# HKU-MedAI/WSI-HGNN

Hardware: AMD Instinct MI355X
Metric: edges/s fwd+bwd HEATNet4, 10k-node/6-rel synth graph, 1->8 MI355X (higher is better)
Workload: dtype f32 (fp16x3 emulation: 2-way fp16 split scaled per row (Y = XW^T, dX) or per column (dW), 3 products - bf16x6 for small launches; fp32-class error)

## Files before the change

### include/wsi_hgnn.h

```cpp
#ifndef WSI_HGNN_H
#define WSI_HGNN_H

#include <stdint.h>

#ifdef __cplusplus
extern "C" {
#endif

#define WSI_OK        0
#define WSI_EINVAL  (-22)
#define WSI_ENOSYS  (-38)
#define WSI_EFAULT  (-14)
#define WSI_ENOMEM  (-12)

#define WSI_ABI_VERSION 26

int         wsi_abi_version(void);
const char* wsi_last_error(void);

typedef struct wsi_context wsi_context_t;
int  wsi_context_create(wsi_context_t** out);
void wsi_context_destroy(wsi_context_t* ctx);

#define WSI_ATTN_XCD_CONTIGUOUS 1
#define WSI_ATTN_HUB_DEGREE(d) (((d) & 0xffff) << 8)
int wsi_heat_attn_fwd(const float* q, int64_t ldq, const float* k, int64_t ldk, const float* v, int64_t ldv,
                      int32_t num_nodes, int32_t D, int32_t H,
                      const int32_t* node_seg, const int32_t* rowptr, const int32_t* src, const float* sim,
                      const int32_t* order, int32_t num_heavy, int32_t flags,
                      const float* e_weight, const float* e_bias,
                      float* t, int64_t ldt, float* score, float* lse,
                      uint32_t* t_absmax,
                      wsi_context_t* ctx, void* stream);

int wsi_heat_attn_scores_fwd(const float* q, int64_t ldq, const float* k, int64_t ldk, int32_t num_nodes, int32_t D, int32_t H,
                             const int32_t* node_seg, const int32_t* rowptr, const int32_t* src, const float* sim,
                             const int32_t* order, int32_t num_heavy, int32_t flags, const float* e_weight, const float* e_bias,
                             float* score, float* lse, wsi_context_t* ctx, void* stream);

int wsi_heat_pool_coeff(const float* score, const float* lse, const int32_t* edge_seg,
                        const int32_t* colptr, const int32_t* csc_eid, const int32_t* csc_dst, const float* inv_rd,
                        const int32_t* row_seg, int32_t segs_per_type, int32_t n_types, int32_t H, int32_t num_src,
                        float* ctab, void* stream);

int wsi_heat_pool_gtab(const float* h, int64_t ldh, int32_t D, int32_t H, const float* y, const float* beta,
                       const int32_t* chunk_row, const int32_t* chunk_seg, int32_t num_chunks,
                       int32_t segs_per_type, int32_t n_types, float* gtab, void* stream);
// ... 176 lines not shown

int wsi_cross_entropy(const float* logits, const int64_t* labels, int32_t B, int32_t C, float* loss, float* dlogits, int32_t* bad_label, void* stream);

int wsi_segment_dot_diff(const float* g, int64_t ldg, const float* a, int64_t lda, const float* b, int64_t ldb,
                         int32_t D, const int32_t* chunk_row, int32_t num_chunks,
                         const int32_t* seg_chunk, int32_t num_segs,
                         float* partial, float* out, void* stream);

int wsi_gate_grad(const float* g, int64_t ldg, const float* a, int64_t lda, const float* b, int64_t ldb,
                  int32_t D, const int32_t* chunk_row, int32_t num_chunks, const int32_t* seg_chunk, int32_t num_segs,
                  const int32_t* seg_gate, const float* skip, int32_t n_gates, float* partial, float* g_skip, void* stream);

int wsi_pool_factors(const float* x, int64_t ldx, int32_t D, const float* w, int64_t ldw, int32_t T, int32_t H, int32_t Bg,
                     const int32_t* chunk_row, int32_t num_chunks, const int32_t* seg_chunk,
                     float* partial, float* hp, float* csum, float* x_mean, void* stream);
int wsi_pool_tmean(const float* tpart, int32_t T, int32_t S, int32_t D, int32_t H, const float* csum, const float* const* bv,
                   const float* scale, float* t_mean, void* stream);
int wsi_pool_bwd_prep(const float* g_pool, int32_t S, int32_t D, int32_t op, const float* counts, const float* z_mean, const float* h_mean,
                      const int32_t* seg_gate, const float* skip, int32_t n_gates, const int32_t* type_gate, int32_t T,
                      float* g_row, float* g_sum, float* g_skip, float* omg, void* stream);
int wsi_pool_bwd_bias(const float* gt_seg, int32_t T, int32_t S, int32_t D, int32_t H, const float* const* bv, const float* csum,
                      float* beta, float* gbv, void* stream);

int wsi_plan_assemble(const int64_t* desc, int32_t nsegs, int32_t total_blocks, void* stream);
int wsi_slot_fill(const int64_t* desc, int32_t nsegs, int32_t total_blocks, void* stream);

int wsi_layernorm_fwd(const float* x, int64_t ldx, int32_t n, int32_t D, float eps,
                      const float* gamma, const float* beta, const int32_t* row_param,
                      float* y, int64_t ldy, float* stats, void* stream);
int wsi_layernorm_bwd(const float* gy, int64_t ldgy, const float* x, int64_t ldx, int32_t n, int32_t D,
                      const float* gamma, const int32_t* row_param, const float* stats,
                      float* gx, int64_t ldgx, float* xhat_gy, int64_t ldp, void* stream);
int wsi_gelu_fwd(const float* x, float* y, int64_t n, void* stream);
int wsi_gelu_bwd(const float* x, const float* gy, float* gx, int64_t n, void* stream);
int wsi_spmm_sum(const float* x, int64_t ldx, int32_t n_out, int32_t D,
                 const int32_t* ptr, const int32_t* idx, const float* edge_w, const float* iscale, const float* oscale,
                 const float* bias, int32_t relu, const float* relu_ref, int64_t ldref,
                 float* out, int64_t ldo, void* stream);
int wsi_sddmm_dot(const float* g, int64_t ldg, const float* x, int64_t ldx, int32_t n, int32_t D,
                  const int32_t* rowptr, const int32_t* src, const float* iscale, const float* oscale,
                  const float* relu_ref, int64_t ldref, float* g_w, void* stream);

int wsi_row_sqnorm(const float* x, int64_t ldx, int32_t n, int32_t F, float* out, void* stream);
int wsi_knn_select(const float* dots, int64_t ldd, const float* sqnorm, int32_t row0, int32_t rows, int32_t N,
                   int32_t kc, int32_t* cand, void* stream);
int wsi_pair_stats(const float* x, int64_t ldx, int32_t n, int32_t F, const int32_t* cand, int32_t kc, int32_t keep,
// ... 83 lines not shown
```

### wsi-hgnn_amd/csrc/heat_attn.hip

```cpp
#include "common.h"
#include <math.h>
#include <stdlib.h>
#include <mutex>
#include <type_traits>
#include <new>

namespace wsi {

struct AttnGraph {
    const int32_t* node_seg;
    const int32_t* rowptr;
    const int32_t* src;
    const float* sim;
    const int32_t* order;
    int32_t num_nodes;
    int32_t heavy_n;
    int32_t pass;
    int32_t heavy_deg;
    int32_t xcd;
    uint32_t* absmax;
    const float* score_in;
    const int32_t* gt_row;
};

// ... 342 lines not shown
    const float* __restrict__ score, const float* __restrict__ lse, const int32_t* __restrict__ edge_seg,
    const int32_t* __restrict__ colptr, const int32_t* __restrict__ csc_eid, const int32_t* __restrict__ csc_dst,
    const float* __restrict__ inv_rd, const int32_t* __restrict__ row_seg, int32_t segs_per_type, int32_t n_types, int32_t H,
    int32_t num_src, float* __restrict__ ctab) {
    const int64_t idx = (int64_t)blockIdx.x * 256 + threadIdx.x;
    if (idx >= (int64_t)num_src * H) return;
    const int u = (int)(idx / H), h = (int)(idx - (int64_t)u * H);
    float cb[kPoolTypes];
#pragma unroll
    for (int b = 0; b < kPoolTypes; ++b) cb[b] = 0.f;
    const int j0 = colptr[u], j1 = colptr[u + 1];
    for (int j = j0; j < j1; ++j) {
        const int e = csc_eid[j], w = csc_dst[j];
        const float a = expf(score[(int64_t)e * H + h] - lse[(int64_t)edge_seg[e] * H + h]) * inv_rd[w];
        const int bin = row_seg[w] / segs_per_type;
#pragma unroll
        for (int b = 0; b < kPoolTypes; ++b) cb[b] += (bin == b) ? a : 0.f;
    }
#pragma unroll
    for (int b = 0; b < kPoolTypes; ++b)
        if (b < n_types) ctab[((int64_t)u * n_types + b) * H + h] = cb[b];
}

template <int V, int LPH, int U, bool COOP = false>
__global__ __launch_bounds__(kBlock) void heat_attn_bwd_p2_kernel(
    AttnTables tb, AttnGraph g, const float* __restrict__ e_weight, const float* __restrict__ e_bias,
    float inv_sqrt_dk, const float* __restrict__ a, const float* __restrict__ ga,
    float* __restrict__ gsc, float* __restrict__ gea, float* __restrict__ gq, int64_t ldgq) {
    constexpr int H = 64 / LPH;
    __shared__ float sm_acc[COOP ? kWavesPerBlock * 64 * V : 1];
    int lane;
    const int w = wave_uniform_node<COOP>(g, lane);
    if (w < 0) return;
    const int part = COOP ? (int)(threadIdx.x >> 6) : 0;
    constexpr int ESTEP = COOP ? kWavesPerBlock * U : U;
    const int head = lane / LPH;
    const bool leader = (lane % LPH) == 0;
    const int col = lane * V;

    float gqa[V];
#pragma unroll
    for (int i = 0; i < V; ++i) gqa[i] = 0.f;

    const int s0 = g.node_seg[w], s1 = g.node_seg[w + 1];
    if (s1 > s0 && g.rowptr[s0] != g.rowptr[s1]) {
        float q[V];
        load_vec<V>(q, tb.q + (int64_t)w * tb.ldq + col);
        const float we = *e_weight, be = *e_bias;
        for (int s = s0; s < s1; ++s) {
            const int e0 = g.rowptr[s], e1 = g.rowptr[s + 1];
            if (e0 == e1) continue;
            float delta = 0.f;
            for (int e = e0; e < e1; ++e) {
                const int64_t o = (int64_t)e * H + head;
                delta = fmaf(a[o], ga[o], delta);
            }
            for (int e = e0 + part * U; e < e1; e += ESTEP) {
                float kk[U][V];
                float c[U], aa[U], gg[U];
#pragma unroll
                for (int j = 0; j < U; ++j) {
                    if (e + j < e1) {
                        const int u = g.src[e + j];
                        c[j] = (we * g.sim[e + j] + be) * inv_sqrt_dk;
                        const int64_t o = (int64_t)(e + j) * H + head;
                        aa[j] = a[o];
                        gg[j] = ga[o];
                        load_vec<V>(kk[j], tb.k + (int64_t)u * tb.ldk + col);
                    }
                }
#pragma unroll
                for (int j = 0; j < U; ++j) {
                    if (e + j < e1) {
                        float d = 0.f;
#pragma unroll
                        for (int i = 0; i < V; ++i) d = fmaf(q[i], kk[j][i], d);
                        d = group_sum<LPH>(d);
                        const float gs = aa[j] * (gg[j] - delta);
                        const float gc = gs * c[j];
#pragma unroll
                        for (int i = 0; i < V; ++i) gqa[i] = fmaf(gc, kk[j][i], gqa[i]);
                        if (leader) {
                            const int64_t o = (int64_t)(e + j) * H + head;
                            gsc[o] = gc;
                            gea[o] = gs * d * inv_sqrt_dk;
                        }
                    }
                }
            }
        }
    }
    if constexpr (COOP) {
#pragma unroll
        for (int i = 0; i < V; ++i) sm_acc[(part * V + i) * 64 + lane] = gqa[i];
        __syncthreads();
        if (part != 0) return;
#pragma unroll
        for (int i = 0; i < V; ++i) {
            float x = 0.f;
#pragma unroll
// ... 25 lines not shown
    int u = order ? order[wave] : wave;
    u = __builtin_amdgcn_readfirstlane(u);
    const int head = lane / LPH;
    const int col = lane * V;

    float gka[V], gva[V];
#pragma unroll
    for (int i = 0; i < V; ++i) { gka[i] = 0.f; gva[i] = 0.f; }
    float cb[POOL ? kPoolTypes : 1];
#pragma unroll
    for (int b = 0; b < (POOL ? kPoolTypes : 1); ++b) cb[b] = 0.f;

    const int j0 = colptr[u], j1 = colptr[u + 1];
    for (int j = j0; j < j1; j += U) {
        float qq[U][V], gt[U][V];
        float aa[U], gg[U];
        int bin[U];
#pragma unroll
        for (int x = 0; x < U; ++x) {
            if (j + x < j1) {
                const int eid = csc_eid[j + x];
                const int w = csc_dst[j + x];
                const int64_t o = (int64_t)eid * H + head;
                if constexpr (!KONLY) aa[x] = a[o] * inv_rd[w];
                gg[x] = gsc[o];
                load_vec<V>(qq[x], qtab + (int64_t)w * ldq + col);
                if constexpr (POOL) bin[x] = pool.ctab_ready ? -1 : pool.row_seg[w] / pool.segs_per_type;
                else if constexpr (!KONLY) load_vec<V>(gt[x], g_t + (int64_t)(gt_row ? gt_row[w] : w) * ldgt + col);
            }
        }
#pragma unroll
        for (int x = 0; x < U; ++x) {
            if (j + x < j1) {
#pragma unroll
                for (int i = 0; i < V; ++i) {
                    gka[i] = fmaf(gg[x], qq[x][i], gka[i]);
                    if constexpr (!POOL && !KONLY) gva[i] = fmaf(aa[x], gt[x][i], gva[i]);
                }
                if constexpr (POOL) {
#pragma unroll
                    for (int b = 0; b < kPoolTypes; ++b) cb[b] += (bin[x] == b) ? aa[x] : 0.f;
                }
            }
        }
    }
    store_vec<V>(gk + (int64_t)u * ldgk + col, gka);
    if constexpr (POOL) {
        const int su = pool.row_seg[u];
        const int tu = su / pool.segs_per_type, gu = su - tu * pool.segs_per_type;
        float racc[V];
        load_vec<V>(racc, pool.g_row + (int64_t)su * (V * 64) + col);
        const float om = pool.omg[tu];
#pragma unroll
        for (int i = 0; i < V; ++i) racc[i] *= om;
        const float* ybase = pool.y + (int64_t)tu * pool.num_segs * H * (V * 64);
#pragma unroll
        for (int b = 0; b < kPoolTypes; ++b) {
            if (b < pool.n_types) {
                if (pool.ctab_ready) cb[b] = pool.ctab[((int64_t)u * pool.n_types + b) * H + head];
                const float* yrow = ybase + (int64_t)(b * pool.segs_per_type + gu) * H * (V * 64) + col;
#pragma unroll
                for (int h = 0; h < H; ++h) {
                    const float c = __shfl(cb[b], h * LPH, 64);
                    float yv[V];
// ... 489 lines not shown
        AttnGraph gh = g, gl = g;
        gh.pass = 2; gh.num_nodes = g.heavy_n;
        gl.pass = 1;
        SideStream* side;
        hipStream_t hs = hub_fork(st, ctx, side);
        hipLaunchKernelGGL((heat_attn_fwd_kernel<V, LPH, kHeavyUnroll, true, true>), dim3(g.heavy_n), dim3(kBlock), 0, hs,
                           tb, gh, ew, eb, isd, (float*)nullptr, (int64_t)0, score, lse);
        hipLaunchKernelGGL((heat_attn_fwd_kernel<V, LPH, U, false, true>), dim3(blocks), dim3(kBlock), 0, st,
                           tb, gl, ew, eb, isd, (float*)nullptr, (int64_t)0, score, lse);
        hub_join(st, side);
        return check_launch("heat_attn_scores_fwd");
    }
    hipLaunchKernelGGL((heat_attn_fwd_kernel<V, LPH, U, false, true>), dim3(blocks), dim3(kBlock), 0, st,
                       tb, g, ew, eb, isd, (float*)nullptr, (int64_t)0, score, lse);
    return check_launch("heat_attn_scores_fwd");
}

template <int V, int LPH>
int launch_bwd(const AttnTables& tb, const AttnGraph& gd, int32_t num_src, int32_t E,
               const int32_t* colptr, const int32_t* csc_eid, const int32_t* csc_dst, const float* inv_rd,
               const int32_t* order_src, const float* ew, const float* eb, float isd,
               const float* g_t, int64_t ldgt, float* score_a, const float* lse, float* ga, float* gsc, float* gea,
               float* red_ws, float* gq, int64_t ldgq, float* gk, int64_t ldgk, float* gv, int64_t ldgv,
               float* g_e, const AttnPool* pool, SideStream* ctx, hipStream_t st) {
    constexpr int U = Unroll<V, LPH>::value;
    constexpr int H = 64 / LPH;
    const int blocks = (gd.num_nodes + kWavesPerBlock - 1) / kWavesPerBlock;
    const int sblocks = (num_src + kWavesPerBlock - 1) / kWavesPerBlock;
    const bool ph = pool && pool->h;
    const bool pflat = pool && pool->gtab;
    const char* bwd_mode = knob("WSI_ATTN_BWD");
    const bool srcmajor = !pool && !(bwd_mode && bwd_mode[0] == 'd');
    if (srcmajor) {
        int32_t* edge_seg = reinterpret_cast<int32_t*>(gsc);
        if (E > 0)
            hipLaunchKernelGGL(heat_attn_edge_seg_kernel, dim3((unsigned)((E + 255) / 256)), dim3(256), 0, st, gd.node_seg, gd.rowptr, gd.num_nodes, E, edge_seg);
        if (sblocks > 0) {
            constexpr int UA = U;
            auto pass_a = [&](auto uu) {
                hipLaunchKernelGGL((heat_attn_bwd_srcA_kernel<V, LPH, decltype(uu)::value>), dim3(sblocks), dim3(kBlock), 0, st,
                                   tb.v, tb.ldv, g_t, ldgt, gd.gt_row, gd.node_seg, (const int32_t*)edge_seg, colptr, csc_eid, csc_dst, inv_rd,
                                   order_src, num_src, gd.xcd, gd.score_in, score_a, lse, ga, gv, ldgv, gd.absmax);
            };
#ifdef WSI_ABLATE
            const char* su = knob("WSI_ATTN_SRC_U");
            const int ua = su ? su[0] - '0' : UA;
            if (ua == 2) pass_a(std::integral_constant<int, 2>{});
            else if (ua == 4) pass_a(std::integral_constant<int, 4>{});
            else if (ua == 8) pass_a(std::integral_constant<int, 8>{});
            else pass_a(std::integral_constant<int, UA>{});
#else
            pass_a(std::integral_constant<int, UA>{});
#endif
        }
    }
    if (pflat && E > 0) {
        const int64_t EH = (int64_t)E * H;
        hipLaunchKernelGGL(heat_attn_bwd_p1_flat_kernel, dim3((unsigned)((EH + 255) / 256)), dim3(256), 0, st, gd.src, pool->edge_seg, pool->seg_dst,
                           pool->row_seg, pool->segs_per_type, pool->n_types, inv_rd, pool->gtab, lse, EH, (int32_t)H, gd.score_in, score_a, ga);
    }
    if (blocks > 0 && gd.heavy_n > 0) {
        AttnGraph gh = gd, gl = gd;
        gh.pass = 2; gh.num_nodes = gd.heavy_n;
        gl.pass = 1;
        const dim3 hb(gd.heavy_n);
        SideStream* side;
        hipStream_t hs = hub_fork(st, ctx, side);
        if (pflat || srcmajor) {}
        else if (ph) hipLaunchKernelGGL((heat_attn_bwd_p1_kernel<V, LPH, kHeavyUnroll, true, true>), hb, dim3(kBlock), 0, hs, tb, gh, g_t, ldgt, score_a, lse, ga, *pool);
        else hipLaunchKernelGGL((heat_attn_bwd_p1_kernel<V, LPH, kHeavyUnroll, true>), hb, dim3(kBlock), 0, hs, tb, gh, g_t, ldgt, score_a, lse, ga, AttnPool{});
        hipLaunchKernelGGL((heat_attn_bwd_p2_kernel<V, LPH, kHeavyUnroll, true>), hb, dim3(kBlock), 0, hs,
                           tb, gh, ew, eb, isd, (const float*)score_a, (const float*)ga, gsc, gea, gq, ldgq);
        if (pflat || srcmajor) {}
        else if (ph) hipLaunchKernelGGL((heat_attn_bwd_p1_kernel<V, LPH, U, false, true>), dim3(blocks), dim3(kBlock), 0, st, tb, gl, g_t, ldgt, score_a, lse, ga, *pool);
        else hipLaunchKernelGGL((heat_attn_bwd_p1_kernel<V, LPH, U>), dim3(blocks), dim3(kBlock), 0, st, tb, gl, g_t, ldgt, score_a, lse, ga, AttnPool{});
        hipLaunchKernelGGL((heat_attn_bwd_p2_kernel<V, LPH, U>), dim3(blocks), dim3(kBlock), 0, st,
                           tb, gl, ew, eb, isd, (const float*)score_a, (const float*)ga, gsc, gea, gq, ldgq);
        hub_join(st, side);
    } else if (blocks > 0) {
        if (pflat || srcmajor) {}
        else if (ph) hipLaunchKernelGGL((heat_attn_bwd_p1_kernel<V, LPH, U, false, true>), dim3(blocks), dim3(kBlock), 0, st,
                                        tb, gd, g_t, ldgt, score_a, lse, ga, *pool);
        else hipLaunchKernelGGL((heat_attn_bwd_p1_kernel<V, LPH, U>), dim3(blocks), dim3(kBlock), 0, st,
                                tb, gd, g_t, ldgt, score_a, lse, ga, AttnPool{});
        hipLaunchKernelGGL((heat_attn_bwd_p2_kernel<V, LPH, U>), dim3(blocks), dim3(kBlock), 0, st,
                           tb, gd, ew, eb, isd, (const float*)score_a, (const float*)ga, gsc, gea, gq, ldgq);
    }
    if (sblocks > 0 && pool)
        hipLaunchKernelGGL((heat_attn_bwd_p3_kernel<V, LPH, U, true>), dim3(sblocks), dim3(kBlock), 0, st,
                           tb.q, tb.ldq, g_t, ldgt, colptr, csc_eid, csc_dst, inv_rd, order_src, num_src, gd.xcd,
                           (const float*)score_a, (const float*)gsc, gk, ldgk, gv, ldgv, gd.absmax, gd.gt_row, *pool);
    else if (sblocks > 0 && srcmajor) {
        constexpr int UC = U;
        auto pass_c = [&](auto uu) {
            hipLaunchKernelGGL((heat_attn_bwd_p3_kernel<V, LPH, decltype(uu)::value, false, true>), dim3(sblocks), dim3(kBlock), 0, st,
                               tb.q, tb.ldq, g_t, ldgt, colptr, csc_eid, csc_dst, inv_rd, order_src, num_src, gd.xcd,
                               (const float*)score_a, (const float*)gsc, gk, ldgk, gv, ldgv, gd.absmax, gd.gt_row, AttnPool{});
        };
#ifdef WSI_ABLATE
        const char* su = knob("WSI_ATTN_SRC_U");
        const int uc = su ? su[su[0] && su[1] ? 1 : 0] - '0' : UC;
        if (uc == 2) pass_c(std::integral_constant<int, 2>{});
        else if (uc == 4) pass_c(std::integral_constant<int, 4>{});
        else if (uc == 8) pass_c(std::integral_constant<int, 8>{});
        else pass_c(std::integral_constant<int, UC>{});
#else
        pass_c(std::integral_constant<int, UC>{});
#endif
    } else if (sblocks > 0)
// ... 68 lines not shown
    if (reinterpret_cast<uintptr_t>(red_ws) & 7) { set_error("heat_attn_bwd: red_ws must be 8-byte aligned (it holds 512 doubles)"); return WSI_EINVAL; }
    AttnPool ap{};
    if (pool) {
        if (!pool->row_seg || !pool->y || !pool->g_row || !pool->omg || !pool->r_out || !pool->ctab || pool->segs_per_type <= 0 ||
            pool->n_types <= 0 || pool->n_types > kPoolTypes || pool->ldr % 4 != 0 || !aligned16(pool->y) || !aligned16(pool->g_row) ||
            !aligned16(pool->r_out) || num_src != num_nodes) {
            set_error("heat_attn_bwd: bad pool descriptor (1..%d node types, 16-byte aligned tables, num_src == num_nodes)", kPoolTypes);
            return WSI_EINVAL;
        }
        if (pool->h && (!pool->beta || pool->ldh % 4 != 0 || !aligned16(pool->h))) { set_error("heat_attn_bwd: pool.h needs pool.beta and 16-byte aligned rows"); return WSI_EINVAL; }
        ap = AttnPool{pool->row_seg, pool->segs_per_type, pool->n_types, pool->n_types * pool->segs_per_type, pool->y, pool->g_row, pool->omg,
                      pool->r_out, pool->ldr, pool->ctab, pool->ctab_ready, pool->h, pool->ldh, pool->beta, pool->gtab, pool->edge_seg, pool->seg_dst};
        if (pool->gtab && (!pool->edge_seg || !pool->seg_dst)) { set_error("heat_attn_bwd: pool.gtab needs pool.edge_seg and pool.seg_dst"); return WSI_EINVAL; }
    }
    const bool al = (ldq | ldk | (v ? ldv : 0) | ldgt | ldgq | ldgk | (gv ? ldgv : 0)) % 4 == 0 && aligned16(q) && aligned16(k) && aligned16(v) &&
                    aligned16(g_t) && aligned16(gq) && aligned16(gk) && aligned16(gv);
    AttnTables tb{q, ldq, k, ldk, v, ldv};
    if (num_heavy < 0 || num_heavy > num_nodes || (num_heavy > 0 && !order_dst)) { set_error("heat_attn_bwd: bad num_heavy=%d", num_heavy); return WSI_EINVAL; }
    AttnGraph gd{node_seg, rowptr, src, sim, order_dst, num_nodes, num_heavy, 0, heavy_degree(flags), (flags & WSI_ATTN_XCD_CONTIGUOUS) ? 1 : 0, g_absmax, score ? score : score_a, g_t_row};
    const float isd = 1.0f / sqrtf((float)(D / H));
    hipStream_t st = (hipStream_t)stream;
#define CALL(V, LPH) return launch_bwd<V, LPH>(tb, gd, num_src, num_edges, colptr, csc_eid, csc_dst, inv_rd, order_src, e_weight, \
                                               e_bias, isd, g_t, ldgt, score_a, lse, ga, gsc, gea, red_ws, gq, ldgq, gk,  \
                                               ldgk, gv, ldgv, g_e, pool ? &ap : nullptr, ctx, st)
    if (al) { WSI_ATTN_DISPATCH(CALL) }
#undef CALL
    if (pool) { set_error("heat_attn_bwd: the pooled backward needs D in {128, 256, 512}, H | 64 and 16-byte aligned rows (D=%d, H=%d)", D, H); return WSI_ENOSYS; }
    if (D <= 1024 && H <= kHMax) {
#define CALL(NV) return launch_bwd_generic<NV>(tb, gd, num_src, num_edges, D, H, colptr, csc_eid, csc_dst, inv_rd, order_src, e_weight, e_bias, \
                                               isd, g_t, ldgt, score_a, lse, ga, gsc, gea, red_ws, gq, ldgq, gk, ldgk, gv, ldgv, g_e, st)
        WSI_ATTN_GENERIC(CALL)
#undef CALL
    }
    set_error("heat_attn_bwd: unsupported (D=%d, H=%d)", D, H);
    return WSI_ENOSYS;
}

extern "C" int wsi_heat_attn_scores_fwd(const float* q, int64_t ldq, const float* k, int64_t ldk, int32_t num_nodes, int32_t D, int32_t H,
                                        const int32_t* node_seg, const int32_t* rowptr, const int32_t* src, const float* sim,
                                        const int32_t* order, int32_t num_heavy, int32_t flags, const float* e_weight, const float* e_bias,
                                        float* score, float* lse, wsi_context_t* ctx, void* stream) {
    if (num_nodes < 0 || D <= 0 || H <= 0 || D % H != 0) { set_error("heat_attn_scores_fwd: bad shape N=%d D=%d H=%d", num_nodes, D, H); return WSI_EINVAL; }
    if (num_nodes == 0) return WSI_OK;
    if (!q || !k || !node_seg || !rowptr || !e_weight || !e_bias || !score || !lse) { set_error("heat_attn_scores_fwd: null pointer"); return WSI_EINVAL; }
    if (num_heavy < 0 || num_heavy > num_nodes || (num_heavy > 0 && !order)) { set_error("heat_attn_scores_fwd: bad num_heavy=%d", num_heavy); return WSI_EINVAL; }
    const bool al = (ldq | ldk) % 4 == 0 && aligned16(q) && aligned16(k);
    AttnTables tb{q, ldq, k, ldk, nullptr, 0};
// ... 79 lines not shown
```

### wsi-hgnn_amd/csrc/pooled.hip

```cpp
#include "common.h"
#include <math.h>

namespace wsi {

constexpr int POOL_MAX_TYPES = 16;
struct PtrList { const float* p[POOL_MAX_TYPES]; };

__global__ __launch_bounds__(256) void pool_tmean_kernel(const float* __restrict__ tpart, int tau0, int nt, int T, int S, int D, int H,
                                                         const float* __restrict__ csum, const PtrList bv, const float* __restrict__ scale,
                                                         int accumulate, int finish, float* __restrict__ t_mean) {
    const int s = blockIdx.x, c = blockIdx.y * 256 + threadIdx.x;
    if (c >= D) return;
    const int hh = c / (D / H);
    float acc = accumulate ? t_mean[(int64_t)s * D + c] : 0.f;
    for (int i = 0; i < nt; ++i) {
        const int tau = tau0 + i;
        acc += tpart[((int64_t)tau * S + s) * D + c];
        if (bv.p[i]) acc = fmaf(csum[((int64_t)tau * S + s) * H + hh], bv.p[i][c], acc);
    }
    if (finish && scale) acc *= scale[s];
    t_mean[(int64_t)s * D + c] = acc;
}

__global__ __launch_bounds__(256) void pool_bwd_prep_kernel(const float* __restrict__ g_pool, int S, int D, int mean, const float* __restrict__ counts,
// ... 12 lines not shown
        for (int c = lane; c < D; c += 64) {
            const int64_t i = (int64_t)s * D + c;
            const float g = g_pool[i];
            const float gs = g * fs;
            g_row[i] = g * fr;
            g_sum[i] = gs;
            acc = fmaf(gs, z_mean[i] - h_mean[i], acc);
        }
        acc = wave_sum(acc);
        if (lane == 0) dots[s] = acc;
    }
    __syncthreads();
    for (int gt = threadIdx.x; gt < n_gates; gt += 256) {
        float acc = 0.f;
        for (int s = 0; s < S; ++s) acc += (seg_gate[s] == gt) ? dots[s] : 0.f;
        g_skip[gt] = acc * (1.f - 1.f / (1.f + expf(-skip[gt])));
    }
    for (int i = threadIdx.x; i < T; i += 256) {
        const int gt = type_gate[i];
        omg[i] = gt >= 0 ? 1.f - 1.f / (1.f + expf(-skip[gt])) : 1.f;
    }
}

__global__ __launch_bounds__(256) void pool_bwd_bias_kernel(const float* __restrict__ gt_seg, int tau0, int nt, int S, int D, int H, const PtrList bv,
                                                            const float* __restrict__ csum, float* __restrict__ beta, float* __restrict__ gbv) {
    const int dk = D / H;
    int blk = blockIdx.x;
    if (beta) {
        if (blk < nt * S) {
            const int i = blk / S, s = blk - i * S, tau = tau0 + i;
            const int lane = threadIdx.x & 63, wave = threadIdx.x >> 6;
            for (int hh = wave; hh < H; hh += 4) {
                float acc = 0.f;
                if (bv.p[i])
                    for (int c = lane; c < dk; c += 64) acc = fmaf(gt_seg[(int64_t)s * D + hh * dk + c], bv.p[i][hh * dk + c], acc);
                acc = wave_sum(acc);
                if (lane == 0) beta[((int64_t)tau * S + s) * H + hh] = acc;
            }
            return;
        }
        blk -= nt * S;
    }
    if (!gbv) return;
    const int tiles = (D + 255) / 256;
    const int i = blk / tiles, c = (blk - i * tiles) * 256 + threadIdx.x, tau = tau0 + i;
    if (i >= nt || c >= D) return;
    const int hh = c / dk;
    float acc = 0.f;
// ... 12 lines not shown
    hipStream_t st = (hipStream_t)stream;
    for (int t0 = 0; t0 < T; t0 += POOL_MAX_TYPES) {
        const int nt = (T - t0 < POOL_MAX_TYPES) ? T - t0 : POOL_MAX_TYPES;
        PtrList L;
        for (int i = 0; i < POOL_MAX_TYPES; ++i) L.p[i] = (i < nt) ? bv[t0 + i] : nullptr;
        hipLaunchKernelGGL(pool_tmean_kernel, dim3(S, (D + 255) / 256), dim3(256), 0, st, tpart, t0, nt, (int)T, (int)S, (int)D, (int)H, csum, L, scale,
                           t0 > 0 ? 1 : 0, t0 + nt >= T ? 1 : 0, t_mean);
    }
    return check_launch("pool_tmean");
}

extern "C" int wsi_pool_bwd_prep(const float* g_pool, int32_t S, int32_t D, int32_t op, const float* counts, const float* z_mean, const float* h_mean,
                                 const int32_t* seg_gate, const float* skip, int32_t n_gates, const int32_t* type_gate, int32_t T,
                                 float* g_row, float* g_sum, float* g_skip, float* omg, void* stream) {
    if (S <= 0 || S > 8192 || D <= 0 || n_gates <= 0 || T <= 0 || (op != WSI_RED_SUM && op != WSI_RED_MEAN)) { set_error("pool_bwd_prep: bad argument"); return WSI_EINVAL; }
    if (!g_pool || !counts || !z_mean || !h_mean || !seg_gate || !skip || !type_gate || !g_row || !g_sum || !g_skip || !omg) {
        set_error("pool_bwd_prep: null pointer"); return WSI_EINVAL;
    }
    hipLaunchKernelGGL(pool_bwd_prep_kernel, dim3(1), dim3(256), (size_t)S * sizeof(float), (hipStream_t)stream, g_pool, (int)S, (int)D,
                       op == WSI_RED_MEAN ? 1 : 0, counts, z_mean, h_mean, seg_gate, skip, (int)n_gates, type_gate, (int)T, g_row, g_sum, g_skip, omg);
    return check_launch("pool_bwd_prep");
}

extern "C" int wsi_pool_bwd_bias(const float* gt_seg, int32_t T, int32_t S, int32_t D, int32_t H, const float* const* bv, const float* csum,
                                 float* beta, float* gbv, void* stream) {
    if (T <= 0 || S <= 0 || D <= 0 || H <= 0 || D % H) { set_error("pool_bwd_bias: bad argument"); return WSI_EINVAL; }
    if (!gt_seg || (beta && !bv) || (gbv && !csum)) { set_error("pool_bwd_bias: null pointer"); return WSI_EINVAL; }
    if (!beta && !gbv) return WSI_OK;
    hipStream_t st = (hipStream_t)stream;
    const int tiles = (D + 255) / 256;
    for (int t0 = 0; t0 < T; t0 += POOL_MAX_TYPES) {
        const int nt = (T - t0 < POOL_MAX_TYPES) ? T - t0 : POOL_MAX_TYPES;
        PtrList L;
        for (int i = 0; i < POOL_MAX_TYPES; ++i) L.p[i] = (beta && i < nt) ? bv[t0 + i] : nullptr;
        const int blocks = (beta ? nt * S : 0) + (gbv ? nt * tiles : 0);
        hipLaunchKernelGGL(pool_bwd_bias_kernel, dim3(blocks), dim3(256), 0, st, gt_seg, t0, nt, (int)S, (int)D, (int)H, L, csum, beta, gbv);
    }
    return check_launch("pool_bwd_bias");
}
```

### wsi-hgnn_amd/ops.py

```python
from __future__ import annotations

import ctypes
import contextlib
from typing import List, Optional, Sequence, Tuple

import torch

from . import _native as N
from .graph import GraphPlan, SegmentTable, host_to_device



_TIMING = {"on": False, "records": []}


def enable_kernel_timing(on: bool) -> None:
    _TIMING["on"] = bool(on)
    _TIMING["records"] = []


class _Timed:
    def __init__(self, name: str, flops: float = 0.0, mfma_flops: float = 0.0):
        self.name, self.flops, self.mfma_flops = name, flops, mfma_flops

# ... 962 lines not shown
_LOW_RANK = {"enabled": True}


_KQV_LAYOUT = {"order": "kqv"}


def set_kqv_layout(order: str) -> None:
    if order not in ("kqv", "kvq"):
        raise ValueError("kqv layout: 'kqv' or 'kvq'")
    _KQV_LAYOUT["order"] = order


def _kqv_blocks(nproj: int):
    return (0, 2, 1) if (nproj == 3 and _KQV_LAYOUT["order"] == "kvq") else (0, 1, 2)


_COLLAPSE_V = {"enabled": True, "min_work": 4.0e9}


def set_value_collapse(on: bool, min_work: Optional[float] = None) -> None:
    _COLLAPSE_V["enabled"] = bool(on)
    if min_work is not None:
        _COLLAPSE_V["min_work"] = float(min_work)


def set_low_rank_readout_grad(on: bool) -> None:
    _LOW_RANK["enabled"] = bool(on)


class _SegmentReduce(torch.autograd.Function):
    @staticmethod
    def forward(ctx, x, rp: ReducePlan, op: int):
        N.require_cuda(x)
        x = x.contiguous()
        out, argmax = _segment_reduce_raw(x, rp, op)
        ctx.rp, ctx.op, ctx.shape = rp, op, x.shape
        ctx.x_id = (x.data_ptr(), x._version)
        ctx.save_for_backward(argmax) if argmax is not None else ctx.save_for_backward(out)
        return out

    @staticmethod
    def backward(ctx, gout):
        lib = N.load()
        rp, op = ctx.rp, ctx.op
        gout = gout.contiguous()
        n, D = ctx.shape
# ... 394 lines not shown
        ctx.save_for_backward(h, kqv, t, out, score, lse, skip, ew, eb, sim_csr, *(() if (drop_mask is None or counter is not None) else (drop_mask,)), *params)
        return out

    @staticmethod
    def backward(ctx, g_out):
        lib = N.load()
        hctx, H, T = ctx.hctx, ctx.H, ctx.T
        bc = None
        if ctx.pool is not None:
            h, kqv, t_mean, h_mean, z_mean, score, lse, skip, ew, eb, sim_csr, *params = ctx.saved_tensors
            fwd_factors = None
            if ctx.no_v:
                fwd_factors, params = params[:3], params[3:]
            t = out = None
            prp, pop = ctx.pool
            n_rows, D_ = h.shape
            pre = None
            segs_p = prp.segments_of(hctx.rows)
            if prp.num_segs <= 8192 and segs_p is not None:
                seg_gate, type_gate = _gate_tables(hctx, skip, segs_p, prp.num_segs)
                g_pool = g_out.contiguous()
                g_row, g_sum = torch.empty_like(g_pool), torch.empty_like(g_pool)
                pre = (torch.empty_like(skip), torch.empty(T, dtype=torch.float32, device=h.device))
                N.check(lib.wsi_pool_bwd_prep(N.ptr(g_pool), prp.num_segs, D_, pop, N.ptr(prp.counts()), N.ptr(z_mean), N.ptr(h_mean), N.ptr(seg_gate),
                                              N.ptr(skip), skip.shape[0], N.ptr(type_gate), T, N.ptr(g_row), N.ptr(g_sum), N.ptr(pre[0]), N.ptr(pre[1]),
                                              N.stream()), "wsi_pool_bwd_prep")
                bc = SegmentBroadcast.from_parts(prp, g_row, g_sum, z_mean)
            else:
                bc = SegmentBroadcast.from_pooled_gradient(g_out.contiguous(), prp, pop, z_mean)
            collapse = ctx.no_v or _value_collapse_applies(hctx, prp, n_rows, D_, H)
            if collapse:
                g_out = None
            else:
                g_out = torch.empty((n_rows, D_), dtype=torch.float32, device=h.device)
                N.check(lib.wsi_segment_reduce_bwd(N.ptr(bc.g_row), D_, D_, N.WSI_RED_SUM, N.ptr(prp.chunk_row), N.ptr(prp.chunk_seg),
                                                   prp.num_chunks, N.ptr(prp.seg_chunk), prp.num_segs, None,
                                                   N.ptr(g_out), D_, N.stream()), "wsi_segment_reduce_bwd")
        else:
            h, kqv, t, out, score, lse, skip, ew, eb, sim_csr, *params = ctx.saved_tensors
            t_mean = h_mean = None
            collapse = False
            fwd_factors = None
            pre = None
            g_out = g_out.contiguous()
        g_y = g_out
        if ctx.has_mask and getattr(ctx, "counter", None) is not None:
            g_y = dropout_apply(g_out, ctx.counter)
        elif ctx.has_mask:
            g_y = g_out * params[0]
# ... 117 lines not shown
            S, dk = bc.rp.num_segs, D // H
            from .graph import host_to_device
            ytab = torch.empty((T, S, H, D), dtype=torch.float32, device=dev)
            groups = []
            for tau in range(T):
                for hh in range(H):
                    groups.append(dict(A=N.ptr(gt_seg, hh * dk * 4), lda=D, B=N.ptr(P[tau][2], hh * dk * D * 4), ldb=D,
                                       C=N.ptr(ytab, ((tau * S) * H + hh) * D * 4), ldc=H * D, M=S, N=D, K=dk))
            _gemm(N.WSI_GEMM_NN, 0, groups, dev)
            if pre is not None:
                omg = pre[1]
            else:
                qt = hctx.cache.get("gate_of_row_type")
                if qt is None:
                    qt = hctx.cache["gate_of_row_type"] = host_to_device(
                        [[1.0 if (hctx.incoming[i] and hctx.nid[i] == g_) else 0.0 for g_ in range(skip.shape[0])] for i in range(T)], torch.float32, dev).view(T, -1)
                omg = 1.0 - qt @ (sig_skip if sig_skip is not None else torch.sigmoid(skip))
            r_out = torch.empty((n, D), dtype=torch.float32, device=dev)
            bv_ptrs = _ptr_array([P[tau][6] for tau in range(T)])
            gbv = torch.empty((T, D), dtype=torch.float32, device=dev)
            if no_v:
                ctab, hp, csum = fwd_factors
                beta = torch.empty((T, S, H), dtype=torch.float32, device=dev)
                N.check(lib.wsi_pool_bwd_bias(N.ptr(gt_seg), T, S, D, H, bv_ptrs, N.ptr(csum), N.ptr(beta), N.ptr(gbv), N.stream()), "wsi_pool_bwd_bias")
            else:
                ctab = torch.empty((n, T, H), dtype=torch.float32, device=dev)
                beta = None
            gtab = None
            if no_v and T * H <= 32 and T * H * (D + 4) * 4 <= 64 * 1024:
                gtab = torch.empty((n, T, H), dtype=torch.float32, device=dev)
                with _Timed("heat_attn"), _Timed("heat_attn_bwd_pooled"):
                    N.check(lib.wsi_heat_pool_gtab(N.ptr(h), D, D, H, N.ptr(ytab), N.ptr(beta), N.ptr(bc.rp.chunk_row), N.ptr(bc.rp.chunk_seg),
                                                   bc.rp.num_chunks, S // T, T, N.ptr(gtab), N.stream()), "wsi_heat_pool_gtab")
            pool_desc = N.AttnPool(row_seg=N.ptr(bc.rp.row_segment()), segs_per_type=S // T, n_types=T, y=N.ptr(ytab), g_row=N.ptr(bc.g_row),
                                   omg=N.ptr(omg), r_out=N.ptr(r_out), ldr=D, ctab=N.ptr(ctab), ctab_ready=1 if no_v else 0,
                                   h=N.ptr(h) if no_v else None, ldh=D, beta=N.ptr(beta), gtab=N.ptr(gtab),
                                   edge_seg=N.ptr(_edge_segments(plan)) if gtab is not None else None,
                                   seg_dst=N.ptr(_segment_dst(plan)) if gtab is not None else None)
            pool_arg = ctypes.byref(pool_desc)
        _background_flush(dev)
        with _Timed("heat_attn"), _Timed("heat_attn_bwd_pooled" if collapse else "heat_attn_bwd_full"):
            N.check(lib.wsi_heat_attn_bwd(
                N.ptr(kqv, qO), ldp, N.ptr(kqv, kO), ldp, None if no_v else N.ptr(kqv, vO), ldp, n, plan.num_src_rows, E, D, H,
                N.ptr(plan.node_seg), N.ptr(plan.rowptr), N.ptr(plan.src), N.ptr(sim_csr),
                N.ptr(plan.colptr), N.ptr(plan.csc_eid), N.ptr(plan.csc_dst),
                N.ptr(plan.inv_rd), N.ptr(plan.order_dst), plan.num_heavy, N.ptr(plan.order_src), _attn_flags(plan), N.ptr(ew), N.ptr(eb),
                N.ptr(g_t), D, N.ptr(gt_row), N.ptr(score), N.ptr(a), N.ptr(lse), N.ptr(scratch[0]), N.ptr(scratch[1]), N.ptr(scratch[2]), N.ptr(red_ws),
                N.ptr(gkqv, qO), ldp, N.ptr(gkqv, kO), ldp, None if no_v else N.ptr(gkqv, vO), ldp,
                N.ptr(g_e), N.ptr(gkqv_max), pool_arg, N.context(), N.stream()), "wsi_heat_attn_bwd")
        gk_side = _col_stats_side(gkqv, hctx.rows, dev) if (want_col_stats(n, D, D) and (D % 32 == 0)) else None
        g_h = torch.empty((n, D), dtype=torch.float32, device=dev)
        chunked = (D % 32 == 0)
        nproj = 2 if collapse else 3
        gh_cols = ColStats.allocate(hctx.rows, D, dev, sums=True) if (chunked and want_col_stats(n, D, D)) else None
        gh_wrote = True
        if collapse:
            groups = []
            for i, (r0, r1) in enumerate(hctx.rows):
                groups.append(dict(A=N.ptr(gkqv, r0 * ldp * 4), lda=ldp, B=N.ptr(P[i][0]), B1=N.ptr(P[i][1]), b_chunk=D, ldb=D, Bw=[P[i][0], P[i][1]],
                                   C=N.ptr(g_h, r0 * D * 4), ldc=D, R=N.ptr(r_out, r0 * D * 4), ldr=D, M=r1 - r0, N=D, K=2 * D,
                                   **_scale_in(gkqv_max, r0), **_scale_out(gh_max, r0),
                                   **(gh_cols.produce(r0, r1, 0) if gh_cols is not None else {})))
            gh_wrote = _gemm(N.WSI_GEMM_NN, N.WSI_EPI_ADD_R, groups, dev)
        for with_gate in ((True, False) if not collapse else ()):
            idxs = [i for i in range(T) if hctx.incoming[i] == with_gate]
            if not idxs:
                continue
            epi = N.WSI_EPI_ADD_R | (N.WSI_EPI_R_1MG if with_gate else 0)
            if chunked:
# ... 818 lines not shown
```

Baseline: 111.7 million.

## Fuse pooled-readout backward chain: lookup attention grads in p2, fold gate tail into bias kernel

```diff
diff --git a/include/wsi_hgnn.h b/include/wsi_hgnn.h
--- a/include/wsi_hgnn.h
+++ b/include/wsi_hgnn.h
@@ -23,6 +23,7 @@
 void wsi_context_destroy(wsi_context_t* ctx);
 
 #define WSI_ATTN_XCD_CONTIGUOUS 1
+#define WSI_ATTN_POOL_LOOKUP_IN_P2 2
 #define WSI_ATTN_HUB_DEGREE(d) (((d) & 0xffff) << 8)
 int wsi_heat_attn_fwd(const float* q, int64_t ldq, const float* k, int64_t ldk, const float* v, int64_t ldv,
                       int32_t num_nodes, int32_t D, int32_t H,
@@ -245,6 +246,12 @@
 int wsi_pool_bwd_bias(const float* gt_seg, int32_t T, int32_t S, int32_t D, int32_t H, const float* const* bv, const float* csum,
                       float* beta, float* gbv, void* stream);
 
+int wsi_pool_bwd_prep_rows(const float* g_pool, int32_t S, int32_t D, int32_t op, const float* counts, const float* z_mean, const float* h_mean,
+                           float* g_row, float* g_sum, float* dots, void* stream);
+int wsi_pool_bwd_bias_gates(const float* gt_seg, int32_t T, int32_t S, int32_t D, int32_t H, const float* const* bv, const float* csum,
+                            float* beta, float* gbv, const float* dots, const int32_t* seg_gate, const float* skip, int32_t n_gates,
+                            const int32_t* type_gate, float* g_skip, float* omg, void* stream);
+
 int wsi_plan_assemble(const int64_t* desc, int32_t nsegs, int32_t total_blocks, void* stream);
 int wsi_slot_fill(const int64_t* desc, int32_t nsegs, int32_t total_blocks, void* stream);
 
diff --git a/wsi-hgnn_amd/csrc/heat_attn.hip b/wsi-hgnn_amd/csrc/heat_attn.hip
--- a/wsi-hgnn_amd/csrc/heat_attn.hip
+++ b/wsi-hgnn_amd/csrc/heat_attn.hip
@@ -388,11 +388,18 @@
         if (b < n_types) ctab[((int64_t)u * n_types + b) * H + h] = cb[b];
 }
 
-template <int V, int LPH, int U, bool COOP = false>
+struct P2Lookup {
+    const float* lse; const float* inv_rd; const float* gtab; const int32_t* row_seg; int32_t segs_per_type, n_types;
+};
+__device__ __forceinline__ float mul_rounded(float x, float y) {
+#pragma clang fp contract(off)
+    return x * y;
+}
+template <int V, int LPH, int U, bool COOP = false, bool LOOKUP = false>
 __global__ __launch_bounds__(kBlock) void heat_attn_bwd_p2_kernel(
     AttnTables tb, AttnGraph g, const float* __restrict__ e_weight, const float* __restrict__ e_bias,
     float inv_sqrt_dk, const float* __restrict__ a, const float* __restrict__ ga,
-    float* __restrict__ gsc, float* __restrict__ gea, float* __restrict__ gq, int64_t ldgq) {
+    float* __restrict__ gsc, float* __restrict__ gea, float* __restrict__ gq, int64_t ldgq, P2Lookup lk) {
     constexpr int H = 64 / LPH;
     __shared__ float sm_acc[COOP ? kWavesPerBlock * 64 * V : 1];
     int lane;
@@ -413,13 +420,33 @@
         float q[V];
         load_vec<V>(q, tb.q + (int64_t)w * tb.ldq + col);
         const float we = *e_weight, be = *e_bias;
+        const int tb_w = LOOKUP ? lk.row_seg[w] / lk.segs_per_type : 0;
+        const float ird = LOOKUP ? lk.inv_rd[w] : 0.f;
         for (int s = s0; s < s1; ++s) {
             const int e0 = g.rowptr[s], e1 = g.rowptr[s + 1];
             if (e0 == e1) continue;
             float delta = 0.f;
-            for (int e = e0; e < e1; ++e) {
-                const int64_t o = (int64_t)e * H + head;
-                delta = fmaf(a[o], ga[o], delta);
+            float ls = 0.f;
+            if constexpr (LOOKUP) {
+                ls = lk.lse[(int64_t)s * H + head];
+                for (int e = e0; e < e1; e += 4) {
+                    float pa[4], pg[4];
+#pragma unroll
+                    for (int j = 0; j < 4; ++j) {
+                        if (e + j < e1) {
+                            pa[j] = g.score_in[(int64_t)(e + j) * H + head];
+                            pg[j] = lk.gtab[((int64_t)g.src[e + j] * lk.n_types + tb_w) * H + head];
+                        }
+                    }
+#pragma unroll
+                    for (int j = 0; j < 4; ++j)
+                        if (e + j < e1) delta = fmaf(expf(pa[j] - ls), mul_rounded(pg[j], ird), delta);
+                }
+            } else {
+                for (int e = e0; e < e1; ++e) {
+                    const int64_t o = (int64_t)e * H + head;
+                    delta = fmaf(a[o], ga[o], delta);
+                }
             }
             for (int e = e0 + part * U; e < e1; e += ESTEP) {
                 float kk[U][V];
@@ -430,8 +457,13 @@
                         const int u = g.src[e + j];
                         c[j] = (we * g.sim[e + j] + be) * inv_sqrt_dk;
                         const int64_t o = (int64_t)(e + j) * H + head;
-                        aa[j] = a[o];
-                        gg[j] = ga[o];
+                        if constexpr (LOOKUP) {
+                            aa[j] = g.score_in[o];
+                            gg[j] = lk.gtab[((int64_t)u * lk.n_types + tb_w) * H + head];
+                        } else {
+                            aa[j] = a[o];
+                            gg[j] = ga[o];
+                        }
                         load_vec<V>(kk[j], tb.k + (int64_t)u * tb.ldk + col);
                     }
                 }
@@ -442,6 +474,10 @@
 #pragma unroll
                         for (int i = 0; i < V; ++i) d = fmaf(q[i], kk[j][i], d);
                         d = group_sum<LPH>(d);
+                        if constexpr (LOOKUP) {
+                            aa[j] = expf(aa[j] - ls);
+                            gg[j] = mul_rounded(gg[j], ird);
+                        }
                         const float gs = aa[j] * (gg[j] - delta);
                         const float gc = gs * c[j];
 #pragma unroll
@@ -513,7 +549,8 @@
                 const int eid = csc_eid[j + x];
                 const int w = csc_dst[j + x];
                 const int64_t o = (int64_t)eid * H + head;
-                if constexpr (!KONLY) aa[x] = a[o] * inv_rd[w];
+                if constexpr (POOL) aa[x] = pool.ctab_ready ? 0.f : a[o] * inv_rd[w];
+                else if constexpr (!KONLY) aa[x] = a[o] * inv_rd[w];
                 gg[x] = gsc[o];
                 load_vec<V>(qq[x], qtab + (int64_t)w * ldq + col);
                 if constexpr (POOL) bin[x] = pool.ctab_ready ? -1 : pool.row_seg[w] / pool.segs_per_type;
@@ -529,8 +566,10 @@
                     if constexpr (!POOL && !KONLY) gva[i] = fmaf(aa[x], gt[x][i], gva[i]);
                 }
                 if constexpr (POOL) {
-#pragma unroll
-                    for (int b = 0; b < kPoolTypes; ++b) cb[b] += (bin[x] == b) ? aa[x] : 0.f;
+                    if (!pool.ctab_ready) {
+#pragma unroll
+                        for (int b = 0; b < kPoolTypes; ++b) cb[b] += (bin[x] == b) ? aa[x] : 0.f;
+                    }
                 }
             }
         }
@@ -1066,13 +1105,15 @@
                const int32_t* order_src, const float* ew, const float* eb, float isd,
                const float* g_t, int64_t ldgt, float* score_a, const float* lse, float* ga, float* gsc, float* gea,
                float* red_ws, float* gq, int64_t ldgq, float* gk, int64_t ldgk, float* gv, int64_t ldgv,
-               float* g_e, const AttnPool* pool, SideStream* ctx, hipStream_t st) {
+               float* g_e, const AttnPool* pool, bool lookup_in_p2, SideStream* ctx, hipStream_t st) {
     constexpr int U = Unroll<V, LPH>::value;
     constexpr int H = 64 / LPH;
     const int blocks = (gd.num_nodes + kWavesPerBlock - 1) / kWavesPerBlock;
     const int sblocks = (num_src + kWavesPerBlock - 1) / kWavesPerBlock;
     const bool ph = pool && pool->h;
     const bool pflat = pool && pool->gtab;
+    const bool plook = pflat && lookup_in_p2 && pool->ctab_ready;
+    const P2Lookup lk = plook ? P2Lookup{lse, inv_rd, pool->gtab, pool->row_seg, pool->segs_per_type, pool->n_types} : P2Lookup{};
     const char* bwd_mode = knob("WSI_ATTN_BWD");
     const bool srcmajor = !pool && !(bwd_mode && bwd_mode[0] == 'd');
     if (srcmajor) {
@@ -1098,7 +1139,7 @@
 #endif
         }
     }
-    if (pflat && E > 0) {
+    if (pflat && !plook && E > 0) {
         const int64_t EH = (int64_t)E * H;
         hipLaunchKernelGGL(heat_attn_bwd_p1_flat_kernel, dim3((unsigned)((EH + 255) / 256)), dim3(256), 0, st, gd.src, pool->edge_seg, pool->seg_dst,
                            pool->row_seg, pool->segs_per_type, pool->n_types, inv_rd, pool->gtab, lse, EH, (int32_t)H, gd.score_in, score_a, ga);
@@ -1113,13 +1154,17 @@
         if (pflat || srcmajor) {}
         else if (ph) hipLaunchKernelGGL((heat_attn_bwd_p1_kernel<V, LPH, kHeavyUnroll, true, true>), hb, dim3(kBlock), 0, hs, tb, gh, g_t, ldgt, score_a, lse, ga, *pool);
         else hipLaunchKernelGGL((heat_attn_bwd_p1_kernel<V, LPH, kHeavyUnroll, true>), hb, dim3(kBlock), 0, hs, tb, gh, g_t, ldgt, score_a, lse, ga, AttnPool{});
-        hipLaunchKernelGGL((heat_attn_bwd_p2_kernel<V, LPH, kHeavyUnroll, true>), hb, dim3(kBlock), 0, hs,
-                           tb, gh, ew, eb, isd, (const float*)score_a, (const float*)ga, gsc, gea, gq, ldgq);
+        if (plook) hipLaunchKernelGGL((heat_attn_bwd_p2_kernel<V, LPH, kHeavyUnroll, true, true>), hb, dim3(kBlock), 0, hs,
+                                      tb, gh, ew, eb, isd, (const float*)nullptr, (const float*)nullptr, gsc, gea, gq, ldgq, lk);
+        else hipLaunchKernelGGL((heat_attn_bwd_p2_kernel<V, LPH, kHeavyUnroll, true>), hb, dim3(kBlock), 0, hs,
+                                tb, gh, ew, eb, isd, (const float*)score_a, (const float*)ga, gsc, gea, gq, ldgq, lk);
         if (pflat || srcmajor) {}
         else if (ph) hipLaunchKernelGGL((heat_attn_bwd_p1_kernel<V, LPH, U, false, true>), dim3(blocks), dim3(kBlock), 0, st, tb, gl, g_t, ldgt, score_a, lse, ga, *pool);
         else hipLaunchKernelGGL((heat_attn_bwd_p1_kernel<V, LPH, U>), dim3(blocks), dim3(kBlock), 0, st, tb, gl, g_t, ldgt, score_a, lse, ga, AttnPool{});
-        hipLaunchKernelGGL((heat_attn_bwd_p2_kernel<V, LPH, U>), dim3(blocks), dim3(kBlock), 0, st,
-                           tb, gl, ew, eb, isd, (const float*)score_a, (const float*)ga, gsc, gea, gq, ldgq);
+        if (plook) hipLaunchKernelGGL((heat_attn_bwd_p2_kernel<V, LPH, U, false, true>), dim3(blocks), dim3(kBlock), 0, st,
+                                      tb, gl, ew, eb, isd, (const float*)nullptr, (const float*)nullptr, gsc, gea, gq, ldgq, lk);
+        else hipLaunchKernelGGL((heat_attn_bwd_p2_kernel<V, LPH, U>), dim3(blocks), dim3(kBlock), 0, st,
+                                tb, gl, ew, eb, isd, (const float*)score_a, (const float*)ga, gsc, gea, gq, ldgq, lk);
         hub_join(st, side);
     } else if (blocks > 0) {
         if (pflat || srcmajor) {}
@@ -1127,8 +1172,10 @@
                                         tb, gd, g_t, ldgt, score_a, lse, ga, *pool);
         else hipLaunchKernelGGL((heat_attn_bwd_p1_kernel<V, LPH, U>), dim3(blocks), dim3(kBlock), 0, st,
                                 tb, gd, g_t, ldgt, score_a, lse, ga, AttnPool{});
-        hipLaunchKernelGGL((heat_attn_bwd_p2_kernel<V, LPH, U>), dim3(blocks), dim3(kBlock), 0, st,
-                           tb, gd, ew, eb, isd, (const float*)score_a, (const float*)ga, gsc, gea, gq, ldgq);
+        if (plook) hipLaunchKernelGGL((heat_attn_bwd_p2_kernel<V, LPH, U, false, true>), dim3(blocks), dim3(kBlock), 0, st,
+                                      tb, gd, ew, eb, isd, (const float*)nullptr, (const float*)nullptr, gsc, gea, gq, ldgq, lk);
+        else hipLaunchKernelGGL((heat_attn_bwd_p2_kernel<V, LPH, U>), dim3(blocks), dim3(kBlock), 0, st,
+                                tb, gd, ew, eb, isd, (const float*)score_a, (const float*)ga, gsc, gea, gq, ldgq, lk);
     }
     if (sblocks > 0 && pool)
         hipLaunchKernelGGL((heat_attn_bwd_p3_kernel<V, LPH, U, true>), dim3(sblocks), dim3(kBlock), 0, st,
@@ -1243,7 +1290,7 @@
     hipStream_t st = (hipStream_t)stream;
 #define CALL(V, LPH) return launch_bwd<V, LPH>(tb, gd, num_src, num_edges, colptr, csc_eid, csc_dst, inv_rd, order_src, e_weight, \
                                                e_bias, isd, g_t, ldgt, score_a, lse, ga, gsc, gea, red_ws, gq, ldgq, gk,  \
-                                               ldgk, gv, ldgv, g_e, pool ? &ap : nullptr, ctx, st)
+                                               ldgk, gv, ldgv, g_e, pool ? &ap : nullptr, (flags & WSI_ATTN_POOL_LOOKUP_IN_P2) != 0, ctx, st)
     if (al) { WSI_ATTN_DISPATCH(CALL) }
 #undef CALL
     if (pool) { set_error("heat_attn_bwd: the pooled backward needs D in {128, 256, 512}, H | 64 and 16-byte aligned rows (D=%d, H=%d)", D, H); return WSI_ENOSYS; }
diff --git a/wsi-hgnn_amd/csrc/pooled.hip b/wsi-hgnn_amd/csrc/pooled.hip
--- a/wsi-hgnn_amd/csrc/pooled.hip
+++ b/wsi-hgnn_amd/csrc/pooled.hip
@@ -58,8 +58,47 @@
     }
 }
 
+__global__ __launch_bounds__(64) void pool_bwd_prep_rows_kernel(const float* __restrict__ g_pool, int S, int D, int mean, const float* __restrict__ counts,
+                                                                const float* __restrict__ z_mean, const float* __restrict__ h_mean,
+                                                                float* __restrict__ g_row, float* __restrict__ g_sum, float* __restrict__ dots) {
+    const int s = blockIdx.x, lane = threadIdx.x;
+    if (s >= S) return;
+    const float cnt = counts[s];
+    const float fr = mean ? (cnt > 0.f ? 1.f / cnt : 0.f) : 1.f;
+    const float fs = mean ? (cnt > 0.f ? 1.f : 0.f) : cnt;
+    float acc = 0.f;
+    for (int c = lane; c < D; c += 64) {
+        const int64_t i = (int64_t)s * D + c;
+        const float g = g_pool[i];
+        const float gs = g * fs;
+        g_row[i] = g * fr;
+        g_sum[i] = gs;
+        acc = fmaf(gs, z_mean[i] - h_mean[i], acc);
+    }
+    acc = wave_sum(acc);
+    if (lane == 0) dots[s] = acc;
+}
+
+struct GateTail {
+    const float* dots; const int32_t* seg_gate; const float* skip; int n_gates; const int32_t* type_gate; int T;
+    float* g_skip; float* omg;
+};
+
 __global__ __launch_bounds__(256) void pool_bwd_bias_kernel(const float* __restrict__ gt_seg, int tau0, int nt, int S, int D, int H, const PtrList bv,
-                                                            const float* __restrict__ csum, float* __restrict__ beta, float* __restrict__ gbv) {
+                                                            const float* __restrict__ csum, float* __restrict__ beta, float* __restrict__ gbv,
+                                                            const GateTail tail) {
+    if (tail.dots && blockIdx.x + 1 == gridDim.x) {
+        for (int gt = threadIdx.x; gt < tail.n_gates; gt += 256) {
+            float acc = 0.f;
+            for (int s = 0; s < S; ++s) acc += (tail.seg_gate[s] == gt) ? tail.dots[s] : 0.f;
+            tail.g_skip[gt] = acc * (1.f - 1.f / (1.f + expf(-tail.skip[gt])));
+        }
+        for (int i = threadIdx.x; i < tail.T; i += 256) {
+            const int gt = tail.type_gate[i];
+            tail.omg[i] = gt >= 0 ? 1.f - 1.f / (1.f + expf(-tail.skip[gt])) : 1.f;
+        }
+        return;
+    }
     const int dk = D / H;
     int blk = blockIdx.x;
     if (beta) {
@@ -118,19 +157,44 @@
     return check_launch("pool_bwd_prep");
 }
 
+static int pool_bwd_bias_launch(const float* gt_seg, int32_t T, int32_t S, int32_t D, int32_t H, const float* const* bv, const float* csum,
+                                float* beta, float* gbv, const GateTail& tail, hipStream_t st) {
+    const int tiles = (D + 255) / 256;
+    for (int t0 = 0; t0 < T; t0 += POOL_MAX_TYPES) {
+        const int nt = (T - t0 < POOL_MAX_TYPES) ? T - t0 : POOL_MAX_TYPES;
+        PtrList L;
+        for (int i = 0; i < POOL_MAX_TYPES; ++i) L.p[i] = (beta && i < nt) ? bv[t0 + i] : nullptr;
+        const GateTail tl = (t0 == 0) ? tail : GateTail{};
+        const int blocks = (beta ? nt * S : 0) + (gbv ? nt * tiles : 0) + (tl.dots ? 1 : 0);
+        hipLaunchKernelGGL(pool_bwd_bias_kernel, dim3(blocks), dim3(256), 0, st, gt_seg, t0, nt, (int)S, (int)D, (int)H, L, csum, beta, gbv, tl);
+    }
+    return check_launch("pool_bwd_bias");
+}
+
 extern "C" int wsi_pool_bwd_bias(const float* gt_seg, int32_t T, int32_t S, int32_t D, int32_t H, const float* const* bv, const float* csum,
                                  float* beta, float* gbv, void* stream) {
     if (T <= 0 || S <= 0 || D <= 0 || H <= 0 || D % H) { set_error("pool_bwd_bias: bad argument"); return WSI_EINVAL; }
     if (!gt_seg || (beta && !bv) || (gbv && !csum)) { set_error("pool_bwd_bias: null pointer"); return WSI_EINVAL; }
     if (!beta && !gbv) return WSI_OK;
-    hipStream_t st = (hipStream_t)stream;
-    const int tiles = (D + 255) / 256;
-    for (int t0 = 0; t0 < T; t0 += POOL_MAX_TYPES) {
-        const int nt = (T - t0 < POOL_MAX_TYPES) ? T - t0 : POOL_MAX_TYPES;
-        PtrList L;
-        for (int i = 0; i < POOL_MAX_TYPES; ++i) L.p[i] = (beta && i < nt) ? bv[t0 + i] : nullptr;
-        const int blocks = (beta ? nt * S : 0) + (gbv ? nt * tiles : 0);
-        hipLaunchKernelGGL(pool_bwd_bias_kernel, dim3(blocks), dim3(256), 0, st, gt_seg, t0, nt, (int)S, (int)D, (int)H, L, csum, beta, gbv);
-    }
-    return check_launch("pool_bwd_bias");
-}
+    return pool_bwd_bias_launch(gt_seg, T, S, D, H, bv, csum, beta, gbv, GateTail{}, (hipStream_t)stream);
+}
+
+extern "C" int wsi_pool_bwd_prep_rows(const float* g_pool, int32_t S, int32_t D, int32_t op, const float* counts, const float* z_mean, const float* h_mean,
+                                      float* g_row, float* g_sum, float* dots, void* stream) {
+    if (S <= 0 || D <= 0 || (op != WSI_RED_SUM && op != WSI_RED_MEAN)) { set_error("pool_bwd_prep_rows: bad argument"); return WSI_EINVAL; }
+    if (!g_pool || !counts || !z_mean || !h_mean || !g_row || !g_sum || !dots) { set_error("pool_bwd_prep_rows: null pointer"); return WSI_EINVAL; }
+    hipLaunchKernelGGL(pool_bwd_prep_rows_kernel, dim3(S), dim3(64), 0, (hipStream_t)stream, g_pool, (int)S, (int)D, op == WSI_RED_MEAN ? 1 : 0, counts,
+                       z_mean, h_mean, g_row, g_sum, dots);
+    return check_launch("pool_bwd_prep_rows");
+}
+
+extern "C" int wsi_pool_bwd_bias_gates(const float* gt_seg, int32_t T, int32_t S, int32_t D, int32_t H, const float* const* bv, const float* csum,
+                                       float* beta, float* gbv, const float* dots, const int32_t* seg_gate, const float* skip, int32_t n_gates,
+                                       const int32_t* type_gate, float* g_skip, float* omg, void* stream) {
+    if (T <= 0 || S <= 0 || D <= 0 || H <= 0 || D % H || n_gates <= 0) { set_error("pool_bwd_bias_gates: bad argument"); return WSI_EINVAL; }
+    if (!gt_seg || (beta && !bv) || (gbv && !csum) || !dots || !seg_gate || !skip || !type_gate || !g_skip || !omg) {
+        set_error("pool_bwd_bias_gates: null pointer"); return WSI_EINVAL;
+    }
+    const GateTail tail{dots, seg_gate, skip, (int)n_gates, type_gate, (int)T, g_skip, omg};
+    return pool_bwd_bias_launch(gt_seg, T, S, D, H, bv, csum, beta, gbv, tail, (hipStream_t)stream);
+}
diff --git a/wsi-hgnn_amd/ops.py b/wsi-hgnn_amd/ops.py
--- a/wsi-hgnn_amd/ops.py
+++ b/wsi-hgnn_amd/ops.py
@@ -1008,6 +1008,13 @@
     _COLLAPSE_V["enabled"] = bool(on)
     if min_work is not None:
         _COLLAPSE_V["min_work"] = float(min_work)
+
+
+_READOUT_CHAIN = {"fused": True}
+
+
+def set_readout_chain_fusion(on: bool) -> None:
+    _READOUT_CHAIN["fused"] = bool(on)
 
 
 def set_low_rank_readout_grad(on: bool) -> None:
@@ -1448,9 +1455,15 @@
                 g_pool = g_out.contiguous()
                 g_row, g_sum = torch.empty_like(g_pool), torch.empty_like(g_pool)
                 pre = (torch.empty_like(skip), torch.empty(T, dtype=torch.float32, device=h.device))
-                N.check(lib.wsi_pool_bwd_prep(N.ptr(g_pool), prp.num_segs, D_, pop, N.ptr(prp.counts()), N.ptr(z_mean), N.ptr(h_mean), N.ptr(seg_gate),
-                                              N.ptr(skip), skip.shape[0], N.ptr(type_gate), T, N.ptr(g_row), N.ptr(g_sum), N.ptr(pre[0]), N.ptr(pre[1]),
-                                              N.stream()), "wsi_pool_bwd_prep")
+                gate_dots = None
+                if ctx.no_v and _READOUT_CHAIN["fused"]:
+                    gate_dots = torch.empty(prp.num_segs, dtype=torch.float32, device=h.device)
+                    N.check(lib.wsi_pool_bwd_prep_rows(N.ptr(g_pool), prp.num_segs, D_, pop, N.ptr(prp.counts()), N.ptr(z_mean), N.ptr(h_mean),
+                                                       N.ptr(g_row), N.ptr(g_sum), N.ptr(gate_dots), N.stream()), "wsi_pool_bwd_prep_rows")
+                else:
+                    N.check(lib.wsi_pool_bwd_prep(N.ptr(g_pool), prp.num_segs, D_, pop, N.ptr(prp.counts()), N.ptr(z_mean), N.ptr(h_mean), N.ptr(seg_gate),
+                                                  N.ptr(skip), skip.shape[0], N.ptr(type_gate), T, N.ptr(g_row), N.ptr(g_sum), N.ptr(pre[0]), N.ptr(pre[1]),
+                                                  N.stream()), "wsi_pool_bwd_prep")
                 bc = SegmentBroadcast.from_parts(prp, g_row, g_sum, z_mean)
             else:
                 bc = SegmentBroadcast.from_pooled_gradient(g_out.contiguous(), prp, pop, z_mean)
@@ -1614,7 +1627,12 @@
             if no_v:
                 ctab, hp, csum = fwd_factors
                 beta = torch.empty((T, S, H), dtype=torch.float32, device=dev)
-                N.check(lib.wsi_pool_bwd_bias(N.ptr(gt_seg), T, S, D, H, bv_ptrs, N.ptr(csum), N.ptr(beta), N.ptr(gbv), N.stream()), "wsi_pool_bwd_bias")
+                if pre is not None and gate_dots is not None:
+                    N.check(lib.wsi_pool_bwd_bias_gates(N.ptr(gt_seg), T, S, D, H, bv_ptrs, N.ptr(csum), N.ptr(beta), N.ptr(gbv), N.ptr(gate_dots),
+                                                        N.ptr(seg_gate), N.ptr(skip), skip.shape[0], N.ptr(type_gate), N.ptr(pre[0]), N.ptr(pre[1]),
+                                                        N.stream()), "wsi_pool_bwd_bias_gates")
+                else:
+                    N.check(lib.wsi_pool_bwd_bias(N.ptr(gt_seg), T, S, D, H, bv_ptrs, N.ptr(csum), N.ptr(beta), N.ptr(gbv), N.stream()), "wsi_pool_bwd_bias")
             else:
                 ctab = torch.empty((n, T, H), dtype=torch.float32, device=dev)
                 beta = None
@@ -1630,13 +1648,14 @@
                                    edge_seg=N.ptr(_edge_segments(plan)) if gtab is not None else None,
                                    seg_dst=N.ptr(_segment_dst(plan)) if gtab is not None else None)
             pool_arg = ctypes.byref(pool_desc)
+        lookup = N.WSI_ATTN_POOL_LOOKUP_IN_P2 if (collapse and no_v and gtab is not None and _READOUT_CHAIN["fused"]) else 0
         _background_flush(dev)
         with _Timed("heat_attn"), _Timed("heat_attn_bwd_pooled" if collapse else "heat_attn_bwd_full"):
             N.check(lib.wsi_heat_attn_bwd(
                 N.ptr(kqv, qO), ldp, N.ptr(kqv, kO), ldp, None if no_v else N.ptr(kqv, vO), ldp, n, plan.num_src_rows, E, D, H,
                 N.ptr(plan.node_seg), N.ptr(plan.rowptr), N.ptr(plan.src), N.ptr(sim_csr),
                 N.ptr(plan.colptr), N.ptr(plan.csc_eid), N.ptr(plan.csc_dst),
-                N.ptr(plan.inv_rd), N.ptr(plan.order_dst), plan.num_heavy, N.ptr(plan.order_src), _attn_flags(plan), N.ptr(ew), N.ptr(eb),
+                N.ptr(plan.inv_rd), N.ptr(plan.order_dst), plan.num_heavy, N.ptr(plan.order_src), _attn_flags(plan) | lookup, N.ptr(ew), N.ptr(eb),
                 N.ptr(g_t), D, N.ptr(gt_row), N.ptr(score), N.ptr(a), N.ptr(lse), N.ptr(scratch[0]), N.ptr(scratch[1]), N.ptr(scratch[2]), N.ptr(red_ws),
                 N.ptr(gkqv, qO), ldp, N.ptr(gkqv, kO), ldp, None if no_v else N.ptr(gkqv, vO), ldp,
                 N.ptr(g_e), N.ptr(gkqv_max), pool_arg, N.context(), N.stream()), "wsi_heat_attn_bwd")
```

Result: no change. 112.7 million, median of 6 (+0.9%).
